# twosigma/Cook

Hardware: AMD Instinct MI355X
Metric: match-cycles/sec at 1M pending x 50k offers (higher is better)
Workload: dtype f64

## Files before the change

### cook_amd/csrc/classfit_walk.hpp

```cpp
#pragma once
#if defined(CF_PROF) && !defined(CF_STATS)
#define CF_STATS 1
#endif
#ifdef CF_STATS
#define CF_STAT(x) x
#define CF_TICKS() cook_ticks()
#else
#define CF_STAT(x) ((void)0)
#define CF_TICKS() 0ull
#endif
#ifdef CF_PROF
#define CF_PROF_T(x) const unsigned long long x = __builtin_readcyclecounter()
#define CF_PROF_ADD(i, d) prof[i] += (unsigned long long)(d)
#else
#define CF_PROF_T(x) ((void)0)
#define CF_PROF_ADD(i, d) ((void)0)
#endif

#ifndef CF_AHEAD
#define CF_AHEAD 10
#endif
constexpr unsigned CF_BOARD = CF_AHEAD;
#ifndef CF_SLOTS_N
#define CF_SLOTS_N 12
#endif
constexpr unsigned CF_SLOTS = CF_SLOTS_N;
static_assert(CF_BOARD + 2u <= CF_SLOTS, "a slot is free again before its wave writes it two rows on");
static_assert(CF_SLOTS == 12u || CF_SLOTS == 24u, "cf_slot and classfit_asm.hpp know these two");
static __device__ __forceinline__ unsigned cf_slot(unsigned ord) { return ord - CF_SLOTS * ((ord * 43u) >> (CF_SLOTS == 12u ? 9 : 10)); }
constexpr unsigned CF_OVL = 58;
constexpr unsigned CF_EPOCH_AT = COOK_SHAPE(58, 8);
constexpr unsigned CFW_BOOKS = 4;
enum : unsigned { CFM_EXACT = 1u, CFM_EPOCH = 2u, CFM_BATCH_END = 3u };
enum : unsigned { CFX_SPARE0 = 0, CFX_SPARE1, CFX_LOGN, CFX_LOG_APPLIED, CFX_WALK_LO, CFX_WALK_HI, CFX_EX_LANE, CFX_FMAX_LO, CFX_FMAX_HI, CFX_EPOCH, CFX_MATCH_LO, CFX_MATCH_HI,
                  CFX_B1_LO, CFX_B1_HI, CFX_OVN, CFX_MINFC, CFX_MINFM, CFX_N = 24 };
constexpr uint32_t CF_ENT_NONE = 0x80000000u, CF_ENT_AMB = 0x40000000u;

struct __attribute__((aligned(8))) CfFree {
  uint32_t c, m;
};
struct CfEnt {
  uint32_t tag, pad, pos, cid;
  uint32_t fc, fm;
  double fa;
};
struct CfLog {
  uint32_t info, pos;
  uint32_t ofc, ofm, nfc, nfm, pad0, pad1;
};
struct CfPost {
  double fa;
  uint32_t w0;
  uint32_t pos;
  uint32_t fc, fm, cls, aux;
};
struct CfJobU {
  unsigned c, m, kind, L, n_eq, n_nov, grouped, grp, eq0, eq1, nov0, nov1;
};
struct CfLds {
  CfFree* fcm;
  uint16_t* cid;
  CfEnt* board;
  CfLog* log;
  uint32_t* ctrl;
  uint64_t* attr8;
  uint16_t *goff, *gcnt, *gids;
  CfJob* ring;
  CfPost* post2;
  CfClass* cls;
  uint32_t* pw;
  uint32_t* aw;
  uint32_t* gk;
  uint32_t* ovt;
  uint32_t* ovl;
  uint32_t* ckept;
  uint32_t* misc;
  const uint32_t* t;
  const uint32_t* envw;
};

static __device__ __forceinline__ unsigned cf_level_of(const uint32_t* t, uint32_t fc) {
  unsigned n = 0;
#pragma unroll
  for (int i = 0; i < CF_LV; ++i) n += fc >= t[i] ? 1u : 0u;
  return n;
}
struct CfLv8 {
// ... 256 lines not shown

template <int ROLE>
static __device__ __forceinline__ void cf_walk_role(const CfLds& S, const MatchState& st, const CfBuf& b, const unsigned lw, const unsigned rep, const unsigned nrep,
                                                    const unsigned long long t_start) {
  constexpr bool is_decider = ROLE == 0, is_class_wave = ROLE == 1, is_books = ROLE == 2;
  const unsigned tid = threadIdx.x, lane = lane_id();
  CfCtl* ctl = b.ctl;
  const unsigned K = wave_uniform_u32(S.envw[CFE_K]), cmin = wave_uniform_u32(S.envw[CFE_CMIN]), mmin = wave_uniform_u32(S.envw[CFE_MMIN]);
  const uint32_t* t = S.t;
#define n_cls wave_uniform_u32(S.envw[CFE_NCLS])
#define n_kind wave_uniform_u32(S.envw[CFE_NKIND])
#define NP wave_uniform_u32(S.envw[CFE_NP])
  CfChunkLane c;
  unsigned nch_wave = 0;
  cf_setup_chunks(S.cls, n_cls, is_class_wave ? lw : 0xFFu, lane, c, nch_wave);
  c.lv = CfLv8{0u, 0u, 0u, 0u, 0u, 0u, 0u, 0u}, c.la = c.lv;
  unsigned my_kinds = 0;
  {
    const unsigned forw = is_class_wave ? lw : (is_decider && lane >= CF_OVL ? lane - CF_OVL + 1u : 0xFFu);
    for (unsigned ci = 0; ci < n_cls; ++ci)
      if (S.cls[ci].wave == forw && S.cls[ci].kind < 32u) my_kinds |= 1u << S.cls[ci].kind;
  }
  const unsigned wk = is_class_wave ? wave_uniform_u32(my_kinds) : 0u;
  unsigned one_cls = 0xFFFFFFFFu, u_off = 0, u_n = 0;
  double u_hTc = 0.0, u_hTm = 0.0;
  auto class_setup = [&] {
    unsigned cnt = 0, ci0 = 0;
    for (unsigned ci = 0; ci < n_cls; ++ci)
      if (S.cls[ci].wave == lw) ++cnt, ci0 = ci;
    one_cls = cnt == 1u ? ci0 : 0xFFFFFFFFu;
    const CfClass* cl = &S.cls[ci0];
    u_off = cl->off, u_n = cl->n, u_hTc = cl->hTc, u_hTm = cl->hTm;
  };
  if (is_class_wave) {
    class_setup();
    for (unsigned ch = 0; ch < nch_wave; ++ch) cf_tighten(S, lane, ch, c);
    if (rep == 0u && lw != 0u) cf_wave_tables(S, lw, lane, c, wk, n_kind);
  }
  CfOvLane o;
  o.valid = 0u, o.id = 0u, o.cls = 0u, o.fc = 0u, o.fm = 0u, o.hTc = 0.0, o.hTm = 0.0;
  unsigned nrm = 0, rm1 = 0xFFFFFFFFu, rm2 = 0xFFFFFFFFu;
  unsigned minfc_all = wave_uniform_u32(S.envw[CFE_MINFC]), minfm_all = wave_uniform_u32(S.envw[CFE_MINFM]);
  unsigned matched = 0, head = 0;
  unsigned jc = 0, jm = 0, jmeta = 0, jgrp = 0, jeq0 = 0, jeq1 = 0, jnov0 = 0, jnov1 = 0;
  int res = -1;
  unsigned long long b1m = 0ull;
  unsigned seen = 0, gen = 0;
  unsigned tight_applied = 0;
  bool bk_room0 = false, nx_room0 = false, nx_walk = false;
  unsigned st_scans = 0, st_exact = 0, st_open = 0, st_ovwin = 0, st_gpu = 0, st_epochs = 0, st_tight = 0, st_walked = 0, st_dead = 0, st_opendead = 0, st_spins = 0, st_flips = 0,
           st_rewinds = 0;
  unsigned long long tk_epoch = 0, tk_books = 0, tk_walk = 0, tk_phase1 = 0;
#ifdef CF_PROF
  unsigned long long prof[8] = {0, 0, 0, 0, 0, 0, 0, 0};
#endif
  auto job_of = [&](unsigned s) -> CfJobU {
    CfJobU J;
    J.c = (unsigned)wave_read_lane((int)jc, (int)s), J.m = (unsigned)wave_read_lane((int)jm, (int)s);
    const unsigned meta = (unsigned)wave_read_lane((int)jmeta, (int)s);
    J.kind = meta & 255u, J.L = (meta >> 8) & 15u, J.n_eq = (meta >> 12) & 15u, J.n_nov = (meta >> 16) & 15u, J.grouped = (meta >> 20) & 1u;
    J.grp = 0u, J.eq0 = J.eq1 = 0u, J.nov0 = J.nov1 = 0xFFFFFFFFu;
    if (meta >> 12) {
      J.grp = (unsigned)wave_read_lane((int)jgrp, (int)s), J.eq0 = (unsigned)wave_read_lane((int)jeq0, (int)s), J.eq1 = (unsigned)wave_read_lane((int)jeq1, (int)s),
      J.nov0 = (unsigned)wave_read_lane((int)jnov0, (int)s), J.nov1 = (unsigned)wave_read_lane((int)jnov1, (int)s);
    }
    return J;
  };
  auto tables_room_any = [&](unsigned L, unsigned m) -> bool {
    bool r = S.ovt[L] > m;
    for (unsigned x = 1; x <= (unsigned)CF_CW; ++x) r = r || S.aw[x * CF_LV + L] > m;
    return r;
  };
  auto tables_walk = [&](unsigned kind, unsigned L, unsigned m) -> bool {
    bool r = false;
    if (kind == 0u) {
      r = S.ovt[L] > m;
      for (unsigned x = 1; x <= (unsigned)CF_CW; ++x) r = r || S.pw[x * CF_LV + L] > m;
    } else if (kind < (unsigned)CF_MAXKIND) {
      r = S.gk[kind * CF_LV + L] > m;
    }
    return r;
  };
  CfJob nxt;
  nxt.c = nxt.m = nxt.meta = nxt.grp = nxt.eq[0] = nxt.eq[1] = nxt.nov[0] = nxt.nov[1] = 0u;
  auto books_next = [&](unsigned nbase) {
    const unsigned nn = nbase < K ? cf_min(64u, K - nbase) : 0u;
    const unsigned nslot = (nbase >> 6) & 1u;
    const bool in = lane < nn;
    if (in) S.ring[nslot * 64u + lane] = nxt;
    const unsigned kind = nxt.meta & 255u, L = (nxt.meta >> 8) & 15u;
    nx_room0 = in && tables_room_any(L, nxt.m);
    nx_walk = in && tables_walk(kind, L, nxt.m);
    const unsigned long long wm = __ballot(nx_walk);
    if (lane == 0)
      S.misc[CFX_WALK_LO] = (unsigned)wm, S.misc[CFX_WALK_HI] = (unsigned)(wm >> 32), S.misc[CFX_LOGN] = 0u, S.misc[CFX_LOG_APPLIED] = 0u,
      S.ctrl[1] = wm ? (unsigned)__ffsll(wm) - 1u : 0u;
  };
  __syncthreads();
  if (is_books) {
    if (lane < cf_min(64u, K)) nxt = b.jobs[lane];
    books_next(0u);
    bk_room0 = nx_room0;
    if (64u + lane < K) nxt = b.jobs[64u + lane];
  }
  if (is_decider) cook_set_prio_high();
  const unsigned long long t_loop = cook_ticks();
  __syncthreads();
  const bool isov = lane < CF_OVL;
  const unsigned clw = isov ? 0u : lane - CF_OVL + 1u;

  for (unsigned base = 0; base < K; base += 64u) {
    const unsigned bn = cf_min(64u, K - base);
    const unsigned slot = (base >> 6) & 1u;
    const unsigned long long walkmask = wave_uniform_u64((unsigned long long)S.misc[CFX_WALK_LO] | (unsigned long long)S.misc[CFX_WALK_HI] << 32);
    const unsigned nw = (unsigned)__popcll(walkmask);
    st_walked += nw;
    if (!is_books) {
      const CfJob j = S.ring[slot * 64u + (lane < bn ? lane : 0u)];
      const bool in = lane < bn;
      jc = in ? j.c : 0u, jm = in ? j.m : 0u, jmeta = in ? j.meta : CF_KIND_NONE, jgrp = j.grp, jeq0 = j.eq[0], jeq1 = j.eq[1], jnov0 = j.nov[0], jnov1 = j.nov[1];
    }
    res = -1;
    if (is_decider) b1m = __ballot(!(jc <= minfc_all && jm <= minfm_all));
    unsigned logn = 0;
    unsigned long long todo = walkmask;
    unsigned cur_ord = 0;
    unsigned ph = 0;
    bool batch_done = nw == 0u;
    const unsigned long long tw0 = CF_TICKS();
    CF_PROF_T(cw0);
    while (!batch_done) {
      unsigned md = 0;
      if (is_decider) {
#if COOK_HAS_ASM_WALK
        cf_u32x16 ST = {0u, 0u, 0u, 0u, 0u, 0u, 0u, 0u, 0u, 0u, 0u, 0u, 0u, 0u, 0u, 0u};
        cf_u32x8 JB = {jc, jm, jmeta, clw * 32u, lane, jeq0, jeq1, 0u};
        const unsigned long long rel0 = cook_ballot(!isov & ((my_kinds & 1u) != 0u)), ovm = cf_below(CF_OVL);
        const cf_u32x8 MK = {wave_uniform_u32((unsigned)rel0), wave_uniform_u32((unsigned)(rel0 >> 32)), wave_uniform_u32((unsigned)ovm), wave_uniform_u32((unsigned)(ovm >> 32)),
                             wave_uniform_u32(cook_lds_off(S.attr8)), 0u, 0u, 0u};
        const unsigned a_board = wave_uniform_u32(cook_lds_off(S.board)), a_log = wave_uniform_u32(cook_lds_off(S.log));
        auto st_pack = [&] {
          const unsigned long long hc = (unsigned long long)__double_as_longlong(o.hTc), hm = (unsigned long long)__double_as_longlong(o.hTm);
          ST[0] = o.valid, ST[1] = o.id, ST[2] = (unsigned)hc, ST[3] = (unsigned)(hc >> 32), ST[4] = (unsigned)hm, ST[5] = (unsigned)(hm >> 32), ST[6] = o.cls, ST[7] = o.fc, ST[8] = o.fm,
          ST[9] = nrm, ST[10] = rm1, ST[11] = rm2, ST[12] = (unsigned)res;
        };
        auto st_unpack = [&] {
          o.valid = ST[0], o.id = ST[1], o.hTc = __longlong_as_double((long long)((unsigned long long)ST[3] << 32 | ST[2])),
          o.hTm = __longlong_as_double((long long)((unsigned long long)ST[5] << 32 | ST[4])), o.cls = ST[6], o.fc = ST[7], o.fm = ST[8], nrm = ST[9], rm1 = ST[10], rm2 = ST[11],
          res = (int)ST[12];
        };
#endif
        while (md == 0u) {
          todo = wave_uniform_u64(todo), cur_ord = wave_uniform_u32(cur_ord), logn = wave_uniform_u32(logn), matched = wave_uniform_u32(matched), gen = wave_uniform_u32(gen);
          minfc_all = wave_uniform_u32(minfc_all), minfm_all = wave_uniform_u32(minfm_all), b1m = wave_uniform_u64(b1m);
#if COOK_HAS_ASM_WALK
          {
            st_pack();
            CF_PROF_T(f0);
            while (todo != 0ull) {
              const unsigned fs = (unsigned)__ffsll(todo) - 1u;
#define CF_U(x) wave_uniform_u32((unsigned)(x))
              cf_u32x8 SC = {CF_U(matched), CF_U(minfc_all), CF_U(b1m), CF_U(b1m >> 32), CF_U(minfm_all), 1u, 0u, 0u};
              const cf_u32x8 AR = {CF_U(fs), CF_U((base + fs) << 12 | (gen & 15u) << 8), CF_U(a_board + cf_slot(cur_ord) * 8u * (unsigned)sizeof(CfEnt)), CF_U(fs | cur_ord << 8),
                                   CF_U(a_log + logn * (unsigned)sizeof(CfLog)), CF_U(cmin), CF_U(mmin), a_board};
#undef CF_U
              asm volatile(CF_ASM_DECIDER_STEP
                           : "+{v[64:79]}"(ST), "+{s[36:43]}"(SC)
                           : "{v[80:87]}"(JB), "{s[44:51]}"(AR), "{s[52:59]}"(MK)
                           : "v88", "v89", "v90", "v91", "v92", "v93", "v94", "v95", "v96", "v97", "v98", "v99", "v100", "v101", "v102", "v103", "v104", "v105", "v106", "v107", "v108",
                             "v109", "v110", "v111", "v112", "v113", "v114", "v115", "v116", "v117", "v118", "v119", "s60", "s61", "s62", "s63", "s64", "s65", "s66", "s67", "s68", "s69",
                             "s70", "s71", "s72", "s73", "s74", "s75", "s76", "s77", "s78", "s79", "s80", "s81", "s82", "s83", "vcc", "scc", "memory");
#ifdef CF_DELAY_D
              __builtin_amdgcn_s_sleep(6);
#endif
              const unsigned status = wave_uniform_u32(SC[5]);
              if (status == 1u) break;
              matched = wave_uniform_u32(SC[0]), minfc_all = wave_uniform_u32(SC[1]), minfm_all = wave_uniform_u32(SC[4]);
              b1m = wave_uniform_u64((unsigned long long)SC[3] << 32 | SC[2]);
              logn += status >> 1;
              todo &= todo - 1ull, ++cur_ord;
              CF_PROF_ADD(4, 1);
            }
            CF_PROF_T(f1);
            CF_PROF_ADD(5, f1 - f0);
            WAIT_LDS();
            st_unpack();
          }
#endif
          if (todo == 0ull) {
            md = CFM_BATCH_END;
            st_lane0_b32(&S.ctrl[0], md);
            break;
          }
          CF_PROF_T(p0);
          const unsigned s = (unsigned)__ffsll(todo) - 1u;
          const unsigned ord = cur_ord;
          st_lane0_b32(&S.ctrl[1], s | ord << 8);
          const unsigned Jc = (unsigned)wave_read_lane((int)jc, (int)s), Jm = (unsigned)wave_read_lane((int)jm, (int)s), meta = (unsigned)wave_read_lane((int)jmeta, (int)s);
          const unsigned kind = meta & 255u;
          const unsigned want = (base + s) << 12 | (gen & 15u) << 8;
          const CfEnt* e = &S.board[cf_slot(ord) * 8u + clw];
          const bool relevant = !isov && kind < 32u && ((my_kinds >> (kind & 31u)) & 1u);
          unsigned cpos, ccid, cfc, cfm;
          double cfa;
          bool acc;
          bool ok_ov = isov & (o.valid != 0u) & (kind == 0u) & (o.fc >= Jc) & (o.fm >= Jm);
          if (meta >> 12) {
            const CfJobU J = job_of(s);
            ok_ov = ok_ov & cf_cons_ok(S, J, o.id, ok_ov);
          }
          for (;;) {
            const unsigned t1 = ld_wg(&e->tag);
            COMPILER_FENCE();
            cpos = e->pos, ccid = e->cid, cfc = e->fc, cfm = e->fm, cfa = e->fa;
            COMPILER_FENCE();
            const unsigned t2 = ld_wg(&e->tag);
            const unsigned behind = (nrm - t1) & 255u, p = cpos & 0xFFFFu;
            const bool ours = (t1 == t2) & ((t1 & ~255u) == want);
            acc = ours & (((ccid & CF_ENT_NONE) != 0u) | ((behind <= 2u) & (p != rm1) & (p != rm2)));
            if (cook_ballot(relevant & !acc) == 0ull) break;
            for (unsigned long long rq = cook_ballot(relevant & !acc & ours); rq != 0ull; rq &= rq - 1ull) {
              const unsigned L = (unsigned)__ffsll(rq) - 1u;
              const unsigned xid = (unsigned)wave_read_lane((int)(ccid & CF_IDMASK), (int)L);
              if (cook_ballot(ok_ov & (o.id == xid)) != 0ull && lane == L) acc = true, ccid = CF_ENT_NONE;
            }
            if (cook_ballot(relevant & !acc) == 0ull) break;
            CF_STAT(++st_spins);
            SPIN_PAUSE_NEAR();
          }
          CF_PROF_T(p1);
          CF_PROF_ADD(0, p1 - p0);
          const unsigned vfc = isov ? o.fc : cfc, vfm = isov ? o.fm : cfm, vid = isov ? o.id : (ccid & CF_IDMASK);
          const bool vvalid = isov ? (o.valid != 0u && kind == 0u) : (relevant && !(ccid & CF_ENT_NONE));
          const bool room = vvalid & (vfc >= Jc) & (vfm >= Jm);
          const bool ok = isov ? ok_ov : room;
          double fov = 1.0 - ((double)(vfc - Jc) * o.hTc + (double)(vfm - Jm) * o.hTm);
          OPAQUE_V(fov);
          const double fa = ok ? (isov ? fov : cfa) : 0.0;
          const float ff = (float)fa;
          const float mx = wave_max_f32(ff);
          const unsigned long long eqm = cook_ballot(ok & (ff == mx)), nearm = cook_ballot(ok & (ff >= mx - CF_BAND32)),
                                   ambm = cook_ballot(ok & !isov & ((ccid & CF_ENT_AMB) != 0u) & (ff >= mx - CF_BAND32));
// ... 191 lines not shown
            }
            CF_PROF_T(q2);
            CF_PROF_ADD(0, q1 - q0);
            CF_PROF_ADD(1, q2 - q1);
            CF_PROF_ADD(3, 1);
          };
          if (cnt != seen) {
            seen = cnt;
            CF_STAT(++st_rewinds);
            unsigned long long t2 = walkmask & ~cf_below(hw & 255u);
            unsigned o2 = hw >> 8, p2 = o2;
            while (p2 >= nrep) p2 -= nrep;
            for (; t2 != 0ull && o2 < cur_ord; t2 &= t2 - 1ull, ++o2, p2 = p2 + 1u == nrep ? 0u : p2 + 1u)
              if (p2 == rep && wk != 0u) answer((unsigned)__ffsll(t2) - 1u, o2, true);
          }
          if (cur_ord < (hw >> 8)) {
            todo = walkmask & ~cf_below(hw & 255u);
            cur_ord = hw >> 8;
            ph = cur_ord;
            while (ph >= nrep) ph -= nrep;
          }
          while (todo != 0ull && ph != rep) {
            todo &= todo - 1ull, ++cur_ord;
            ph = ph + 1u == nrep ? 0u : ph + 1u;
          }
          if (todo != 0ull && wk != 0u && cur_ord < (hw >> 8) + CF_BOARD) {
            const unsigned s = (unsigned)__ffsll(todo) - 1u;
            const unsigned ord = cur_ord;
            todo &= todo - 1ull, ++cur_ord;
            ph = ph + 1u == nrep ? 0u : ph + 1u;
            answer(s, ord, false);
            continue;
          }
          if (wk != 0u) SPIN_PAUSE_NEAR();
          else SPIN_PAUSE_IDLE();
          CF_PROF_T(q4);
          CF_PROF_ADD(4, q4 - q0);
          CF_PROF_ADD(5, 1);
        }
      } else {
        while (md == 0u) {
          const unsigned mode = cf_poll(&S.ctrl[0]);
          if (mode != 0u) {
            md = mode;
            break;
          }
          SPIN_PAUSE_IDLE();
        }
      }
      EMU_SITE("classfit: collective");
      WAIT_LDS();
      __syncthreads();
      md = wave_uniform_u32(md);
      bool epoch = md == CFM_EPOCH;
      const unsigned s = wave_uniform_u32(S.misc[CFX_EX_LANE]);
      if (md == CFM_EXACT) {
        ++st_exact;
        const double fmax = __longlong_as_double((long long)((unsigned long long)S.misc[CFX_FMAX_LO] | (unsigned long long)S.misc[CFX_FMAX_HI] << 32));
        CfPost mine;
        if (is_decider) {
          const CfJobU J = job_of(s);
          cf_overlay_query_exact(S, J, lane, o, fmax, cf_pow2(-(int)wave_uniform_u32(S.envw[CFE_KC])), cf_pow2(-(int)wave_uniform_u32(S.envw[CFE_KM])), mine);
          if (lane == 0) S.post2[0] = mine;
        } else if (is_class_wave && rep == 0u && lw != 0u) {
          const CfJobU J = job_of(s);
          cf_class_query_exact(S, J, lane, c, fmax, cf_pow2(-(int)wave_uniform_u32(S.envw[CFE_KC])), cf_pow2(-(int)wave_uniform_u32(S.envw[CFE_KM])), mine, st_scans);
          if (lane == 0) S.post2[lw] = mine;
        }
        EMU_SITE("classfit: exact turn");
        __syncthreads();
        if (is_decider) {
          const CfJobU J = job_of(s);
          unsigned used_sets = 0;
          for (unsigned ci = 0; ci < n_cls; ++ci) used_sets |= 1u << wave_uniform_u32(S.cls[ci].wave);
          const CfVerdict v = cf_verdict_exact(S.post2, lane, used_sets);
          const unsigned nfc = v.fc - J.c, nfm = v.fm - J.m;
          const bool dead = nfc < cmin || nfm < mmin;
          const bool from_ov = v.src == 0;
          const bool gpu_place = !from_ov && J.kind != 0u;
          const bool opens = !from_ov && !gpu_place && !dead;
          ++matched;
          if (lane == s) res = (int)v.id;
          b1m |= __ballot((jc > nfc) | (jm > nfm)) & ~cf_below(s) & ~(1ull << s);
          minfc_all = cf_min(minfc_all, nfc), minfm_all = cf_min(minfm_all, nfm);
          unsigned live = (unsigned)__popcll(__ballot(isov && o.valid != 0u));
          unsigned lpos = 0, linfo = s;
          if (from_ov) {
            CF_STAT(++st_ovwin);
            if (lane == v.pos) {
              o.fc = nfc, o.fm = nfm;
              if (dead) o.valid = 0u;
            }
            if (dead) --live;
          } else {
            lpos = v.pos, linfo = s | (unsigned)v.src << 8 | v.aux << 12 | (gpu_place ? 1u : 0u) << 20;
            if (lane == CF_OVL - 1u + (unsigned)v.src) {
              if (gpu_place) S.fcm[lpos] = CfFree{nfc, nfm}, S.cid[lpos] = (uint16_t)(S.cid[lpos] | CF_OCC);
              else S.fcm[lpos] = CfFree{0u, 0u};
              ++nrm, rm2 = rm1, rm1 = lpos;
              S.ctrl[1u + (unsigned)v.src] = nrm;
            }
            if (opens) {
              CF_STAT(++st_open);
              const unsigned lf = (unsigned)__ffsll(~__ballot((isov && o.valid != 0u) || !isov)) - 1u;
              const CfClass* cl = &S.cls[v.cls];
              const double hTc2 = cl->hTc, hTm2 = cl->hTm;
// ... 88 lines not shown
                  if (!(Ee < Elast || (Ee == Elast && ide < idlast))) break;
                  const bool before = keep && (Ek < Ee || (Ek == Ee && idq < ide));
                  const unsigned long long bm = __ballot(before);
                  if (keep && !before) ++ins_before;
                  const unsigned np = noff + kept_before + (unsigned)__popcll(bm) + (ip - li);
                  if (lane == 0) st_agent(&b.scr_fc[np], efc), st_agent(&b.scr_fm[np], efm), st_agent(&b.scr_cid[np], ecid);
                  ++ip;
                }
                if (keep) {
                  const unsigned np = noff + kept_before + (unsigned)__popcll(keepm & lanemask_lt()) + ins_before;
                  st_agent(&b.scr_fc[np], fc), st_agent(&b.scr_fm[np], fm), st_agent(&b.scr_cid[np], cid);
                }
                kept_before += (unsigned)__popcll(keepm);
              }
              for (; ip < li + ni; ++ip) {
                const unsigned np = noff + kept_before + (ip - li);
                if (lane == 0) st_agent(&b.scr_fc[np], S.ovl[3u * ip + 1u]), st_agent(&b.scr_fm[np], S.ovl[3u * ip + 2u]), st_agent(&b.scr_cid[np], S.ovl[3u * ip]);
              }
            }
            li += ni;
          }
        }
        drain_stores();
        EMU_SITE("classfit: epoch 3");
        __syncthreads();
        unsigned newM = 0;
        for (unsigned ci = 0; ci < n_cls; ++ci) newM += S.ckept[ci] + S.ckept[CF_MAXCLS + ci];
        for (unsigned q = tid; q < NP; q += CF_THREADS) {
          const bool inq = q < newM;
          const uint32_t fcq = inq ? ld_agent(&b.scr_fc[q]) : 0u, fmq = inq ? ld_agent(&b.scr_fm[q]) : 0u, cq = inq ? ld_agent(&b.scr_cid[q]) : 0u;
          bool tie = false;
          if (q + 1u < newM) {
            const uint32_t fcn = ld_agent(&b.scr_fc[q + 1u]), fmn = ld_agent(&b.scr_fm[q + 1u]), cn = ld_agent(&b.scr_cid[q + 1u]);
            if ((cn >> 16) == (cq >> 16)) {
              const CfClass* cl = &S.cls[cq >> 16];
              tie = (unsigned long long)fcn * cl->Tm + (unsigned long long)fmn * cl->Tc <= (unsigned long long)fcq * cl->Tm + (unsigned long long)fmq * cl->Tc + cl->dE;
            }
          }
          S.fcm[q] = CfFree{fcq, fmq}, S.cid[q] = inq ? (uint16_t)((cq & (CF_OCC | CF_IDMASK)) | (tie ? CF_TIE : 0u)) : (uint16_t)0u;
        }
        if (tid < n_cls) S.cls[tid].n = S.ckept[tid] + S.ckept[CF_MAXCLS + tid], S.cls[tid].off = S.ckept[2 * CF_MAXCLS + tid];
        EMU_SITE("classfit: epoch 4");
        __syncthreads();
        if (is_class_wave) {
          cf_setup_chunks(S.cls, n_cls, lw, lane, c, nch_wave);
          class_setup();
          for (unsigned ch = 0; ch < nch_wave; ++ch) cf_tighten(S, lane, ch, c);
          if (rep == 0u && lw != 0u) cf_wave_tables(S, lw, lane, c, wk, n_kind);
          tight_applied = st_tight;
        }
        if (tid == 0) S.misc[CFX_LOG_APPLIED] = S.misc[CFX_LOGN];
        tk_epoch += CF_TICKS() - te;
      }
      if (md == CFM_BATCH_END) batch_done = true;
      if (md != CFM_BATCH_END) {
        ++gen;
        if (is_class_wave) {
          todo = walkmask & ~cf_below(s) & ~(1ull << s), cur_ord = (unsigned)__popcll(walkmask & cf_below(s)) + 1u;
          ph = cur_ord;
          while (ph >= nrep) ph -= nrep;
        }
      }
      if (tid == 0) st_wg(&S.ctrl[0], 0u);
      EMU_SITE("classfit: collective done");
      __syncthreads();
      if (is_class_wave) seen = cf_poll(&S.ctrl[1u + lw]);
    }
    tk_walk += CF_TICKS() - tw0;
    CF_PROF_T(cw1);
    CF_PROF_ADD(7, cw1 - cw0);
    const unsigned long long tp0 = CF_TICKS();
    if (is_decider) {
      if (lane < bn) st.job_to_offer[base + lane] = res;
      const unsigned long long mm = __ballot(res >= 0);
      if (base == 0u) head = (unsigned)(mm & 1ull);
      const bool live = isov && o.valid != 0u;
      const unsigned nl = live ? cf_level_of(t, o.fc) : 0u;
#define CF_OV_T(i) unsigned v##i = nl > (unsigned)i ? o.fm + 1u : 0u;
      CF_FOR8(CF_OV_T)
#undef CF_OV_T
      wave_max8_u32(v0, v1, v2, v3, v4, v5, v6, v7);
      if (lane == 0) {
        S.misc[CFX_MATCH_LO] = (unsigned)mm, S.misc[CFX_MATCH_HI] = (unsigned)(mm >> 32), S.misc[CFX_B1_LO] = (unsigned)b1m, S.misc[CFX_B1_HI] = (unsigned)(b1m >> 32);
        S.misc[CFX_LOGN] = logn, S.misc[CFX_MINFC] = minfc_all, S.misc[CFX_MINFM] = minfm_all;
#define CF_OV_S(i) S.ovt[i] = v##i;
        CF_FOR8(CF_OV_S)
#undef CF_OV_S
      }
    }
    if (nw != 0u) {
      EMU_SITE("classfit: phase 1");
      __syncthreads();
      if (is_class_wave) {
        const unsigned n_log = wave_uniform_u32(S.misc[CFX_LOGN]), a0 = wave_uniform_u32(S.misc[CFX_LOG_APPLIED]);
        const bool mine_e = lane >= a0 && lane < n_log && ((S.log[lane].info >> 8) & 15u) == lw;
        bool dirty = st_tight != tight_applied;
        for (unsigned long long mm = __ballot(mine_e); mm; mm &= mm - 1ull) {
          const unsigned x = (unsigned)__ffsll(mm) - 1u;
          const CfLog lg = S.log[x];
          const unsigned ch = (lg.info >> 12) & 255u;
          bool retable = ((lg.info >> 20) & 1u) != 0u;
          const unsigned nl = cf_level_of(t, lg.ofc);
#define CF_WAS_MAX(i) retable = retable || (__ballot(lane == ch && (unsigned)i < nl && c.lv.v##i == lg.ofm + 1u) != 0ull);
          CF_FOR8(CF_WAS_MAX)
#undef CF_WAS_MAX
          if (retable) {
            cf_tighten(S, lane, ch, c);
            ++st_tight;
            dirty = true;
          }
        }
        if (dirty && rep == 0u && lw != 0u) cf_wave_tables(S, lw, lane, c, wk, n_kind);
        tight_applied = st_tight;
      }
    }
    EMU_SITE("classfit: phase 2");
    __syncthreads();
    tk_phase1 += CF_TICKS() - tp0;
    if (is_books) {
      const unsigned long long tb0 = CF_TICKS();
      const unsigned long long mm = (unsigned long long)S.misc[CFX_MATCH_LO] | (unsigned long long)S.misc[CFX_MATCH_HI] << 32,
                               bb = (unsigned long long)S.misc[CFX_B1_LO] | (unsigned long long)S.misc[CFX_B1_HI] << 32;
      const unsigned n_log = wave_uniform_u32(S.misc[CFX_LOGN]);
      const CfJob j = S.ring[slot * 64u + (lane < bn ? lane : 0u)];
      const bool unm = lane < bn && !((mm >> lane) & 1ull);
      const unsigned L = (j.meta >> 8) & 15u;
      bool room = unm && tables_room_any(L, j.m);
      const bool flip = unm && !room && bk_room0 && n_log != 0u;
      if (__ballot(flip) != 0ull) {
        ++st_flips;
        for (unsigned x = 0; x < n_log; ++x) {
          const CfLog lg = S.log[x];
          if (flip && (lg.info & 255u) > lane && lg.ofc >= j.c && lg.ofm >= j.m) room = true;
        }
      }
      if (lane < bn && st.fail_code) {
        unsigned fail = 0u;
        if (unm) {
          fail = (((bb >> lane) & 1ull) ? 1u : 0u) | (room ? 2u : 0u);
          if (fail == 0u) fail = 8u;
        }
        st.fail_code[base + lane] = fail;
      }
      books_next(base + 64u);
      bk_room0 = nx_room0;
      if (base + 128u + lane < K) nxt = b.jobs[base + 128u + lane];
      tk_books += CF_TICKS() - tb0;
    }
    EMU_SITE("classfit: batch end");
    __syncthreads();
  }
  if (is_decider) {
    if (lane == 0) {
      st.summary[0] = matched;
      st.summary[1] = (matched == 0u || head) ? 1u : 0u;
      st.summary[2] = st_epochs;
      const unsigned long long t_end = cook_ticks();
      uint32_t* sx = ctl->stats;
      sx[CFS_MATCHED] = matched, sx[CFS_OV_WIN] = st_ovwin, sx[CFS_OPEN] = st_open, sx[CFS_OPEN_DEAD] = st_opendead, sx[CFS_GPU_PLACE] = st_gpu, sx[CFS_EPOCHS] = st_epochs,
      sx[CFS_EXACT] = st_exact, sx[CFS_WALKED] = st_walked, sx[CFS_DEAD_DROP] = st_dead, sx[CFS_BATCHES] = (K + 63u) / 64u, sx[CFS_PRESETTLED] = K - st_walked;
      sx[CFS_TICKS_TOTAL] = (uint32_t)(t_end - t_start), sx[CFS_TICKS_PROLOGUE] = (uint32_t)(t_loop - t_start), sx[CFS_TICKS_EPOCH] = (uint32_t)tk_epoch;
      sx[CFS_TICKS_WALK] = (uint32_t)tk_walk, sx[CFS_TICKS_PHASE1] = (uint32_t)tk_phase1;
      sx[CFS_HWID_DECIDER] = cook_hw_id();
    }
    const unsigned sp = wave_max_u32(!isov ? st_spins : 0u);
    if (lane == 0) ctl->stats[CFS_SPINS] = sp;
  }
  if (is_class_wave && lane == 0) atomicAdd(&ctl->stats[CFS_SCANS], st_scans), atomicAdd(&ctl->stats[CFS_TIGHTEN], st_tight), atomicAdd(&ctl->stats[CFS_REWINDS], st_rewinds);
  if (is_books && lane == 0) ctl->stats[CFS_TICKS_PRECHECK] = (uint32_t)tk_books, ctl->stats[CFS_FLIPS] = st_flips, ctl->stats[CFS_HWID_BOOKS] = cook_hw_id();
#ifdef CF_PROF
  if (lane == 0 && (is_decider || (is_class_wave && lw >= 1u && lw <= 2u && rep == 0u)))
    for (int i = 0; i < 8; ++i) ctl->stats[24 + 8 * (is_decider ? 0u : lw) + i] = (uint32_t)(prof[i] >> 4);
#endif
#undef n_cls
#undef n_kind
#undef NP
}

static __device__ __forceinline__ void cf_walk_pool(char* lds, const MatchIn* __restrict__ inp, const MatchState& st, const CfBuf& b) {
  const unsigned tid = threadIdx.x, lane = lane_id(), w = wave_id();
  CfCtl* ctl = b.ctl;
  const unsigned K = inp->K, M = ctl->M, G = inp->G;
  const unsigned NP = (M + 63u) & ~63u;
  const unsigned long long t_start = cook_ticks();
  const bool any_eq = ctl->any_eq != 0u, any_group = ctl->any_group != 0u;
  __shared__ unsigned s_total, s_wsum[CF_WAVES];
  constexpr unsigned GPT = CF_MAXG / CF_THREADS;
  unsigned gsz[GPT];
  unsigned gsum = 0;
#pragma unroll
  for (unsigned x = 0; x < GPT; ++x) {
    const unsigned g = tid * GPT + x;
    unsigned sz = 0;
    if (any_group && g < G && b.gcount[g] != 0u) sz = (inp->g_run_off ? inp->g_run_off[g + 1] - inp->g_run_off[g] : 0u) + b.gcount[g];
    gsz[x] = sz, gsum += sz;
  }
  unsigned incl = gsum;
  for (unsigned d = 1; d < 64u; d <<= 1) {
    const unsigned y = shfl_up_t<unsigned>(incl, d);
    if (lane >= d) incl += y;
  }
  if (lane == 63u) s_wsum[w] = incl;
  __syncthreads();
  unsigned wbase = 0;
  for (unsigned x = 0; x < w; ++x) wbase += s_wsum[x];
  if (tid == CF_THREADS - 1) s_total = wbase + incl;
  __syncthreads();
  const unsigned Stot = any_group ? s_total : 0u, Gl = any_group ? G : 0u;
  CfLds S;
  {
    CfFixed* F = (CfFixed*)lds;
    S.board = F->board, S.log = F->log, S.ring = F->ring, S.post2 = F->post2, S.cls = F->cls, S.pw = F->pw, S.aw = F->aw, S.gk = F->gk, S.ovt = F->ovt, S.ctrl = F->ctrl, S.ovl = F->ovl,
    S.ckept = F->ckept, S.misc = F->misc, S.t = F->env_t, S.envw = F->envw;
    char* p = lds + sizeof(CfFixed);
    S.fcm = (CfFree*)p, p += NP * 8u;
    S.cid = (uint16_t*)p, p += NP * 2u;
    p = lds + (((unsigned)(p - lds) + 7u) & ~7u);
    S.attr8 = (uint64_t*)p;
    if (any_eq) p += M * 8u;
    S.goff = (uint16_t*)p, p += (Gl + 1u) * 2u;
    S.gcnt = (uint16_t*)p, p += Gl * 2u;
    S.gids = (uint16_t*)p, p += Stot * 2u;
    if ((unsigned)(p - lds) > CF_LDS_BYTES) {
      if (tid == 0) atomicOr(&ctl->inelig, (unsigned)CF_X_SHAPE), st.summary[3] = 0xDEADu;
      return;
    }
  }
#ifdef CF_DIAG_CLEAR_LDS
  for (unsigned x = tid; x < CF_LDS_BYTES / 4u; x += CF_THREADS) ((uint32_t*)lds)[x] = 0u;
  __syncthreads();
#endif
  for (unsigned q = tid; q < NP; q += CF_THREADS) {
    S.fcm[q] = q < M ? CfFree{b.pos_fc[q], b.pos_fm[q]} : CfFree{0u, 0u}, S.cid[q] = q < M ? (uint16_t)b.pos_cid[q] : (uint16_t)0u;
  }
  if (any_eq)
    for (unsigned v = tid; v < M; v += CF_THREADS) S.attr8[v] = b.attr8[v];
  if (any_group) {
    unsigned off = wbase + incl - gsum;
#pragma unroll
// ... 81 lines not shown
```

### cook_amd/csrc/engine.hip

```cpp
#include <hip/hip_runtime.h>
#include <sys/mman.h>
#include <ucontext.h>

#include <algorithm>
#include <atomic>
#include <cmath>
#include <cstdlib>
#include <chrono>
#include <cstring>
#include <limits>
#include <functional>
#include <map>
#include <string>
#include <tuple>
#include <vector>

#include "../../include/cookmatch.h"
#include "common.hpp"
#include "multi.hpp"
#include "considerable_kernels.hpp"
#include "match_kernels.hpp"
#include "match_v2.hpp"
#include "classfit.hpp"
#include "offers_kernels.hpp"
// ... 1280 lines not shown
  static_assert(sizeof(CfCtl) % 4 == 0, "cf_init clears the control block word by word");
  KM<cf_init, 256>(e, "cf_init", std::min(div_up(b.max_host + 1u, 1024u), 512u), b, b.max_host + 1u, std::max(1u, G));
  KM<cf_scan, 256>(e, "cf_scan", div_up(std::max(K, M), 256), in_dev, b, K, M);
  KM<cf_prepare, 1024>(e, "cf_prepare", 1u, in_dev, b, st.jmin, K, M, G, in.host_dup, in.reserved_bits ? 1u : 0u);
  KM<cf_pack_jobs, 256>(e, "cf_pack_jobs", div_up(K, 256), in_dev, b, K);
  static_assert(offsetof(CfCtl, t) <= 512, "the control block's head is read back through the 512-byte scratch");
  pinned_copy(e, e->h_scratch, b.ctl, offsetof(CfCtl, t), hipMemcpyDeviceToHost);
  sync(e);
  CfCtl hc;
  std::memcpy((void*)&hc, e->h_scratch, offsetof(CfCtl, t));
  e->cf_inelig = hc.inelig;
  if (hc.inelig) return false;
  const unsigned NP = (M + 63u) & ~63u;
  const unsigned S = hc.any_group ? e->cf_group_run_total + hc.n_grouped : 0u;
  if (cf_lds_bytes_host(NP, M, hc.any_eq != 0u, hc.any_group ? G : 0u, S) > CF_LDS_BYTES || S > 60000u) {
    e->cf_inelig = CF_X_SHAPE;
    return false;
  }
  ctx.in = in_dev;
  ctx.st = st;
  ctx.b = b;
  return true;
}
void cf_run(cook_engine* lead, cook_engine* const* es, unsigned n, hipStream_t stream) {
  cook_engine* e = lead;
  for (unsigned i0 = 0; i0 < n; i0 += (unsigned)CF_PACK) {
    const unsigned c = std::min<unsigned>(CF_PACK, n - i0);
    CfPack pk{};
    for (unsigned x = 0; x < (unsigned)CF_PACK; ++x) pk.c[x] = es[i0 + (x < c ? x : 0u)]->deferred_cf;
    KLS("cf_walk", stream, cf_walk, c, CF_THREADS, pk);
  }
  for (unsigned i = 0; i < n; ++i) {
    const CfPoolCtx& c = es[i]->deferred_cf;
    const unsigned G = es[i]->last_in.G;
    if (G) KLS("cf_group_chains", stream, cf_group_chains, div_up(G, 256), 256, c.b, c.st, G);
  }
  constexpr size_t SLOT = 16 + 48 * 4;
  if (!lead->h_cf) COOK_HIP(hipHostMalloc((void**)&lead->h_cf, 64 * SLOT, hipHostMallocDefault));
  if (n > 64) lead->fail(COOK_E_INVALID, "cook_cycle_match_multi: at most 64 pools per call");
  for (unsigned i = 0; i < n; ++i) {
    char* slot = lead->h_cf + i * SLOT;
    COOK_HIP(hipMemcpyAsync(slot, es[i]->deferred_cf.st.summary, 16, hipMemcpyDeviceToHost, stream));
    COOK_HIP(hipMemcpyAsync(slot + 16, es[i]->deferred_cf.b.ctl->stats, 48 * 4, hipMemcpyDeviceToHost, stream));
  }
  COOK_HIP(hipStreamSynchronize(stream));
  for (unsigned i = 0; i < n; ++i) {
    cook_engine* x = es[i];
    const unsigned* sum = (const unsigned*)(lead->h_cf + i * SLOT);
    if (sum[3] == 0xDEADu) lead->fail(COOK_E_STATE, "cf_walk: the pool's tables do not fit the workgroup's LDS (the host's check let it through)");
    std::memcpy(x->cf_stats, lead->h_cf + i * SLOT + 16, 48 * 4);
#ifdef CF_PROF
    {
      const uint32_t* q = x->cf_stats;
      std::fprintf(stderr, "CFPROF (x16 shader cycles) decider: slow steps %u (candidates %u evaluation %u commit %u) plain steps %u in %u walk-total %u | class wave 1: poll %u answer %u answers %u idle %u idles %u | class wave 2: poll %u answer %u answers %u idle %u idles %u | walk ticks(100MHz) %u\n", q[27], q[24], q[25], q[26], q[28], q[29], q[31], q[32], q[33], q[35], q[36], q[37], q[40], q[41], q[43], q[44], q[45], q[CFS_TICKS_WALK]);
    }
#endif
    WinCtl c{};
    c.matched = sum[0], c.head_matched = sum[1], c.rounds = sum[2], c.head = x->last_in.K, c.visited_sum = x->cf_stats[CFS_WALKED];
    c.t_seq = x->cf_stats[CFS_TICKS_TOTAL], c.t_setup = x->cf_stats[CFS_TICKS_PROLOGUE];
    x->last_ctl = c;
    x->last_form = 3;
    x->has_deferred_cf = false;
    x->has_deferred = false;
    x->match_done = true;
  }
}

void match_run_device(cook_engine* e, unsigned K, const uint32_t* j_index, bool defer = false) {
  MatchIn in = e->min;
  in.K = K;
  in.j_index = j_index;
  in.good_enough = e->params.good_enough_fitness;
  in.host_lifetime_mins = e->params.host_lifetime_mins;
  const unsigned M = in.M, G = in.G;
  e->last_in = in;
  e->last_in_valid = true;
  MatchState st;
  st.ac = e->m_ac.ensure(M);
  st.am = e->m_am.ensure(M);
  st.acount = e->m_acount.ensure(M);
  st.group_last = e->m_group_last.ensure(G);
  st.job_prev = e->m_job_prev.ensure(K);
  st.job_to_offer = e->m_j2o.ensure(K);
  st.fail_code = e->m_fail.ensure(K);
  st.summary = e->m_summary.ensure(4);
  st.alive = e->m_alive.ensure((M + 63u) / 64u + 1u);
  st.jmin = (const double*)e->m_jmin.ensure(4);
  st.xports = in.has_x ? e->m_xports.ensure(M) : nullptr;
  st.xscal = in.has_x ? e->m_xscal.ensure((size_t)M * COOK_MAX_SCALARS) : nullptr;
  match_init_state(e, st, K, M, G);
  st.cutoff = 0x7FFFFFFF;
  e->has_deferred = false;
  const int algo = e->params.match_algo;
  if (!(algo == 0 || algo == 1 || algo == 2 || algo == 3))
    e->fail(COOK_E_INVALID, "cook_params.match_algo: 0 = engine default (window rounds; class-ordered best fit where the call allows it when six or more engines share the device), 1 = serial sweep, 2 = window rounds, 3 = class-ordered best fit where the call allows it, else window rounds");
  if (defer && !(algo != 1 && K > 0)) defer = false;
  const bool ge = in.good_enough < 1.0;
  if (algo == 1) {
    constexpr int SERIAL_THREADS = COOK_SHAPE(1024, 256);
    auto k_match = match_serial<SERIAL_THREADS>;
    KL("match_serial", k_match, 1, SERIAL_THREADS, in, st);
    e->last_form = 1;
    e->has_deferred_cf = false;
  } else if (K > 0) {
    match_check_offer_count(e, M);
    V2Buf vb;
    const char* rlog_path = std::getenv("COOK_ROUND_LOG");
// ... 1311 lines not shown
```

Measured before the change: 21.22.

## Skip walk-free job batches in books wave and fold batch-end into walk loop

The books wave now loops over consecutive 64-job batches that have no walked job, writing their results (-1 and fail codes) directly and prefetching job rows several batches ahead, then publishes the next base so all waves jump past those batches without a workgroup barrier round each. The decider's end-of-batch bookkeeping moves into the walk loop's batch-end branch, and the separate barrier before phase 1 is removed, so the batch-end signal exits the loop early. This is meant to cut per-batch synchronisation and global-load latency across the many empty batches, at the cost of more registers for the prefetch ring and a more delicate ordering between waves.

```diff
diff --git a/cook_amd/csrc/classfit_walk.hpp b/cook_amd/csrc/classfit_walk.hpp
--- a/cook_amd/csrc/classfit_walk.hpp
+++ b/cook_amd/csrc/classfit_walk.hpp
@@ -32,7 +32,7 @@
 constexpr unsigned CF_EPOCH_AT = COOK_SHAPE(58, 8);
 constexpr unsigned CFW_BOOKS = 4;
 enum : unsigned { CFM_EXACT = 1u, CFM_EPOCH = 2u, CFM_BATCH_END = 3u };
-enum : unsigned { CFX_SPARE0 = 0, CFX_SPARE1, CFX_LOGN, CFX_LOG_APPLIED, CFX_WALK_LO, CFX_WALK_HI, CFX_EX_LANE, CFX_FMAX_LO, CFX_FMAX_HI, CFX_EPOCH, CFX_MATCH_LO, CFX_MATCH_HI,
+enum : unsigned { CFX_NEXT_BASE = 0, CFX_SPARE1, CFX_LOGN, CFX_LOG_APPLIED, CFX_WALK_LO, CFX_WALK_HI, CFX_EX_LANE, CFX_FMAX_LO, CFX_FMAX_HI, CFX_EPOCH, CFX_MATCH_LO, CFX_MATCH_HI,
                   CFX_B1_LO, CFX_B1_HI, CFX_OVN, CFX_MINFC, CFX_MINFM, CFX_N = 24 };
 constexpr uint32_t CF_ENT_NONE = 0x80000000u, CF_ENT_AMB = 0x40000000u;
 
@@ -395,7 +395,7 @@
            st_rewinds = 0;
   unsigned long long tk_epoch = 0, tk_books = 0, tk_walk = 0, tk_phase1 = 0;
 #ifdef CF_PROF
-  unsigned long long prof[8] = {0, 0, 0, 0, 0, 0, 0, 0};
+  unsigned long long prof[8] = {0, 0, 0, 0, 0, 0, 0, 0}, bnd0 = 0ull;
 #endif
   auto job_of = [&](unsigned s) -> CfJobU {
     CfJobU J;
@@ -426,7 +426,9 @@
   };
   CfJob nxt;
   nxt.c = nxt.m = nxt.meta = nxt.grp = nxt.eq[0] = nxt.eq[1] = nxt.nov[0] = nxt.nov[1] = 0u;
-  auto books_next = [&](unsigned nbase) {
+  constexpr unsigned CF_PRE = 3;
+  CfJob pre[CF_PRE];
+  auto books_next = [&](unsigned nbase) -> unsigned long long {
     const unsigned nn = nbase < K ? cf_min(64u, K - nbase) : 0u;
     const unsigned nslot = (nbase >> 6) & 1u;
     const bool in = lane < nn;
@@ -438,6 +440,13 @@
     if (lane == 0)
       S.misc[CFX_WALK_LO] = (unsigned)wm, S.misc[CFX_WALK_HI] = (unsigned)(wm >> 32), S.misc[CFX_LOGN] = 0u, S.misc[CFX_LOG_APPLIED] = 0u,
       S.ctrl[1] = wm ? (unsigned)__ffsll(wm) - 1u : 0u;
+    return wm;
+  };
+  auto books_advance = [&](unsigned nbase) {
+    nxt = pre[0];
+#pragma unroll
+    for (unsigned i = 0; i + 1u < CF_PRE; ++i) pre[i] = pre[i + 1u];
+    if (nbase + 64u * (CF_PRE + 1u) + lane < K) pre[CF_PRE - 1u] = b.jobs[nbase + 64u * (CF_PRE + 1u) + lane];
   };
   __syncthreads();
   if (is_books) {
@@ -445,6 +454,11 @@
     books_next(0u);
     bk_room0 = nx_room0;
     if (64u + lane < K) nxt = b.jobs[64u + lane];
+#pragma unroll
+    for (unsigned i = 0; i < CF_PRE; ++i) {
+      pre[i] = nxt;
+      if (64u * (i + 2u) + lane < K) pre[i] = b.jobs[64u * (i + 2u) + lane];
+    }
   }
   if (is_decider) cook_set_prio_high();
   const unsigned long long t_loop = cook_ticks();
@@ -452,7 +466,7 @@
   const bool isov = lane < CF_OVL;
   const unsigned clw = isov ? 0u : lane - CF_OVL + 1u;
 
-  for (unsigned base = 0; base < K; base += 64u) {
+  for (unsigned base = 0; base < K;) {
     const unsigned bn = cf_min(64u, K - base);
     const unsigned slot = (base >> 6) & 1u;
     const unsigned long long walkmask = wave_uniform_u64((unsigned long long)S.misc[CFX_WALK_LO] | (unsigned long long)S.misc[CFX_WALK_HI] << 32);
@@ -470,8 +484,30 @@
     unsigned cur_ord = 0;
     unsigned ph = 0;
     bool batch_done = nw == 0u;
+    auto decider_books = [&](unsigned n_placed) {
+      if (lane < bn) st.job_to_offer[base + lane] = res;
+      const unsigned long long mm = __ballot(res >= 0);
+      if (base == 0u) head = (unsigned)(mm & 1ull);
+      const bool live = isov && o.valid != 0u;
+      const unsigned nl = live ? cf_level_of(t, o.fc) : 0u;
+#define CF_OV_T(i) unsigned v##i = nl > (unsigned)i ? o.fm + 1u : 0u;
+      CF_FOR8(CF_OV_T)
+#undef CF_OV_T
+      wave_max8_u32(v0, v1, v2, v3, v4, v5, v6, v7);
+      if (lane == 0) {
+        S.misc[CFX_MATCH_LO] = (unsigned)mm, S.misc[CFX_MATCH_HI] = (unsigned)(mm >> 32), S.misc[CFX_B1_LO] = (unsigned)b1m, S.misc[CFX_B1_HI] = (unsigned)(b1m >> 32);
+        S.misc[CFX_LOGN] = n_placed, S.misc[CFX_MINFC] = minfc_all, S.misc[CFX_MINFM] = minfm_all;
+#define CF_OV_S(i) S.ovt[i] = v##i;
+        CF_FOR8(CF_OV_S)
+#undef CF_OV_S
+      }
+    };
     const unsigned long long tw0 = CF_TICKS();
     CF_PROF_T(cw0);
+#ifdef CF_PROF
+    if (is_decider && nw != 0u && bnd0 != 0ull) prof[6] += cw0 - bnd0, bnd0 = 0ull;
+    if (is_class_wave && nw == 0u) prof[6] += 16ull;
+#endif
     while (!batch_done) {
       unsigned md = 0;
       if (is_decider) {
@@ -531,6 +567,10 @@
           }
 #endif
           if (todo == 0ull) {
+#ifdef CF_PROF
+            bnd0 = __builtin_readcyclecounter();
+#endif
+            decider_books(logn);
             md = CFM_BATCH_END;
             st_lane0_b32(&S.ctrl[0], md);
             break;
@@ -828,6 +868,12 @@
       WAIT_LDS();
       __syncthreads();
       md = wave_uniform_u32(md);
+      if (md == CFM_BATCH_END) {
+        batch_done = true;
+        if (tid == 0) st_wg(&S.ctrl[0], 0u);
+        if (is_class_wave) seen = cf_poll(&S.ctrl[1u + lw]);
+        break;
+      }
       bool epoch = md == CFM_EPOCH;
       const unsigned s = wave_uniform_u32(S.misc[CFX_EX_LANE]);
       if (md == CFM_EXACT) {
@@ -1022,8 +1068,7 @@
         if (tid == 0) S.misc[CFX_LOG_APPLIED] = S.misc[CFX_LOGN];
         tk_epoch += CF_TICKS() - te;
       }
-      if (md == CFM_BATCH_END) batch_done = true;
-      if (md != CFM_BATCH_END) {
+      {
         ++gen;
         if (is_class_wave) {
           todo = walkmask & ~cf_below(s) & ~(1ull << s), cur_ord = (unsigned)__popcll(walkmask & cf_below(s)) + 1u;
@@ -1040,27 +1085,8 @@
     CF_PROF_T(cw1);
     CF_PROF_ADD(7, cw1 - cw0);
     const unsigned long long tp0 = CF_TICKS();
-    if (is_decider) {
-      if (lane < bn) st.job_to_offer[base + lane] = res;
-      const unsigned long long mm = __ballot(res >= 0);
-      if (base == 0u) head = (unsigned)(mm & 1ull);
-      const bool live = isov && o.valid != 0u;
-      const unsigned nl = live ? cf_level_of(t, o.fc) : 0u;
-#define CF_OV_T(i) unsigned v##i = nl > (unsigned)i ? o.fm + 1u : 0u;
-      CF_FOR8(CF_OV_T)
-#undef CF_OV_T
-      wave_max8_u32(v0, v1, v2, v3, v4, v5, v6, v7);
-      if (lane == 0) {
-        S.misc[CFX_MATCH_LO] = (unsigned)mm, S.misc[CFX_MATCH_HI] = (unsigned)(mm >> 32), S.misc[CFX_B1_LO] = (unsigned)b1m, S.misc[CFX_B1_HI] = (unsigned)(b1m >> 32);
-        S.misc[CFX_LOGN] = logn, S.misc[CFX_MINFC] = minfc_all, S.misc[CFX_MINFM] = minfm_all;
-#define CF_OV_S(i) S.ovt[i] = v##i;
-        CF_FOR8(CF_OV_S)
-#undef CF_OV_S
-      }
-    }
+    if (is_decider && nw == 0u) decider_books(0u);
     if (nw != 0u) {
-      EMU_SITE("classfit: phase 1");
-      __syncthreads();
       if (is_class_wave) {
         const unsigned n_log = wave_uniform_u32(S.misc[CFX_LOGN]), a0 = wave_uniform_u32(S.misc[CFX_LOG_APPLIED]);
         const bool mine_e = lane >= a0 && lane < n_log && ((S.log[lane].info >> 8) & 15u) == lw;
@@ -1112,13 +1138,33 @@
         }
         st.fail_code[base + lane] = fail;
       }
-      books_next(base + 64u);
+      unsigned nb = base + 64u;
+      unsigned long long nwm = books_next(nb);
+      const unsigned minfc_pub = wave_uniform_u32(S.misc[CFX_MINFC]), minfm_pub = wave_uniform_u32(S.misc[CFX_MINFM]);
+      while (nb < K && nwm == 0ull) {
+        if (nb + lane < K) {
+          st.job_to_offer[nb + lane] = -1;
+          if (st.fail_code) {
+            const unsigned fail = ((nxt.c > minfc_pub || nxt.m > minfm_pub) ? 1u : 0u) | (nx_room0 ? 2u : 0u);
+            st.fail_code[nb + lane] = fail != 0u ? fail : 8u;
+          }
+        }
+        books_advance(nb);
+        nb += 64u;
+        nwm = books_next(nb);
+      }
+      if (lane == 0) S.misc[CFX_NEXT_BASE] = nb;
       bk_room0 = nx_room0;
-      if (base + 128u + lane < K) nxt = b.jobs[base + 128u + lane];
+      books_advance(nb);
       tk_books += CF_TICKS() - tb0;
     }
     EMU_SITE("classfit: batch end");
     __syncthreads();
+    const unsigned nbase = wave_uniform_u32(S.misc[CFX_NEXT_BASE]);
+#ifdef CF_PROF
+    if (is_class_wave) prof[6] += 16ull * ((nbase - base) / 64u - 1u);
+#endif
+    base = nbase;
   }
   if (is_decider) {
     if (lane == 0) {
@@ -1155,6 +1201,7 @@
   const unsigned long long t_start = cook_ticks();
   const bool any_eq = ctl->any_eq != 0u, any_group = ctl->any_group != 0u;
   __shared__ unsigned s_total, s_wsum[CF_WAVES];
+  static_assert(CF_MAXG % CF_THREADS == 0, "the groups are dealt out GPT to a thread: a workgroup size that does not divide CF_MAXG would leave some without one");
   constexpr unsigned GPT = CF_MAXG / CF_THREADS;
   unsigned gsz[GPT];
   unsigned gsum = 0;
diff --git a/cook_amd/csrc/engine.hip b/cook_amd/csrc/engine.hip
--- a/cook_amd/csrc/engine.hip
+++ b/cook_amd/csrc/engine.hip
@@ -1356,7 +1356,7 @@
 #ifdef CF_PROF
     {
       const uint32_t* q = x->cf_stats;
-      std::fprintf(stderr, "CFPROF (x16 shader cycles) decider: slow steps %u (candidates %u evaluation %u commit %u) plain steps %u in %u walk-total %u | class wave 1: poll %u answer %u answers %u idle %u idles %u | class wave 2: poll %u answer %u answers %u idle %u idles %u | walk ticks(100MHz) %u\n", q[27], q[24], q[25], q[26], q[28], q[29], q[31], q[32], q[33], q[35], q[36], q[37], q[40], q[41], q[43], q[44], q[45], q[CFS_TICKS_WALK]);
+      std::fprintf(stderr, "CFPROF (x16 shader cycles) decider: slow steps %u (candidates %u evaluation %u commit %u) plain steps %u in %u walk-total %u | class wave 1: poll %u answer %u answers %u idle %u idles %u | class wave 2: poll %u answer %u answers %u idle %u idles %u | walk ticks(100MHz) %u | batch boundaries: decider %u, batches without a walked job %u\n", q[27], q[24], q[25], q[26], q[28], q[29], q[31], q[32], q[33], q[35], q[36], q[37], q[40], q[41], q[43], q[44], q[45], q[CFS_TICKS_WALK], q[30], q[38]);
     }
 #endif
     WinCtl c{};
```

Measured after the change: 21.65, median of 6. 1.02x the previous value.
